# isl-org/Open3D-PointNet2-Semantic3D

Hardware: AMD Instinct MI355X
Metric: points/sec through SA+FP stack (B=16,N=8192) (higher is better)
Workload: dtype f32

## Files before the change

include/pn2_abi.h:

```cpp
#ifndef PN2_ABI_H_
#define PN2_ABI_H_

#include <stddef.h>
#include <stdint.h>

#ifdef __cplusplus
extern "C" {
#endif

#define PN2_ABI_VERSION 1

#define PN2_OK 0
#define PN2_EINVAL (-1)
#define PN2_ENULL (-2)
#define PN2_ERANGE (-3)
#define PN2_EUNSUP (-4)

#define PN2_ARITH_STRICT 0
#define PN2_ARITH_FMA 1
#define PN2_ARITH_FMA_ALT 2

int pn2_abi_version(void);
const char *pn2_build_info(void);
const char *pn2_strerror(int code);
// ... 207 lines not shown
                            double half_y, double scene_z_size, int cap, int *out_idx, int *out_cnt,
                            void *stream);

int pn2_scene_sample(int b, int npts, int cap, const double *points, const int *labels, const double *colors,
                     const int *idx, const int *cnt, const unsigned char *mask, double half_x, double half_y,
                     int *out_sel, float *out_centered, double *out_raw, int *out_labels, float *out_colors,
                     int *status, void *stream);

size_t pn2_voxel_downsample_workspace_bytes(int n);
int pn2_voxel_downsample(int n, const double *points, const double *colors, const int *labels, double voxel_size,
                         double *out_points, double *out_colors, int *out_labels, int *out_count, int *status,
                         void *workspace, size_t workspace_bytes, void *stream);

int pn2_dataset_workspace_size(int b, int max_chunks, unsigned long long *bytes);
int pn2_dataset_sample(int b, int npts, int num_scenes, int max_chunks, int use_color, int augment, const double *points,
                       const float *colors, const unsigned char *labels, const int *scene_offsets, const double *scene_cdf,
                       const double *scene_z_size, const float *label_weights, int num_label_weights, double half_x,
                       double half_y, unsigned long long seed, long long *counter, const int *draw_scene,
                       const int *draw_center, const unsigned char *draw_mask, int mask_cap, const double *draw_rot,
                       void *workspace, size_t workspace_bytes, int *out_info, double *out_finfo, int *out_sel,
                       float *out_data, int *out_labels, float *out_weights, void *stream);

int pn2_fp_mlp_fused_pre(int b, int n, int m, int c1, const float *dist, const int *idx, const float *points1,
                         const float *z, int nlayers, const int *widths, const float *const *w,
                         const float *const *bias, float *y, void *stream);
int pn2_fp_mlp_fused_pre_ld(int b, int n, int m, int c1, const float *dist, const int *idx, const float *points1,
                            int ld_points1, const float *z, int nlayers, const int *widths, const float *const *w,
                            const float *const *bias, float *y, void *stream);

int pn2_fp_mlp_fused_pre_schedule(int b, int n, int m, int c1, const float *dist, const int *idx, const float *points1,
                                  const float *z, int nlayers, const int *widths, const float *const *w,
                                  const float *const *bias, float *y, int schedule, void *stream);

int pn2_sa_mlp_fused_pre(int b, int n, int m, int nsample, const float *xyz, const float *new_xyz, const float *zf,
                         const int *idx, int nlayers, const int *widths, const float *const *w,
                         const float *const *bias, int pool, float *out, void *stream);

int pn2_fp_mlp_wide_pre(int b, int n, int m, int c1, const float *dist, const int *idx, const float *points1,
                        const float *z, int nlayers, const int *widths, const float *const *w,
                        const float *const *bias, float *y, void *stream);
int pn2_sa_mlp_wide_pre(int b, int n, int m, int nsample, const float *xyz, const float *new_xyz, const float *zf,
                        const int *idx, int nlayers, const int *widths, const float *const *w,
                        const float *const *bias, int pool, float *y, void *stream);

size_t pn2_ball_query_bin_bytes(int n);
int pn2_ball_query_bin(int b, int n, float radius, const float *xyz1, void *workspace, size_t workspace_bytes, void *stream);
int pn2_ball_query_bin_ld(int b, int n, float radius, const float *xyz1, int ld1, void *workspace, size_t workspace_bytes,
                          void *stream);
int pn2_query_ball_point_binned(int b, int n, int m, float radius, int nsample, const float *xyz1, const float *xyz2,
                                const void *bins, int *idx, int *pts_cnt, int arith_mode, void *stream);

int pn2_group_pool(long long rows, int k, int c, int mode, const float *x, const float *gxyz, float *out, void *stream);
int pn2_group_pool_grad(long long rows, int k, int c, int mode, const float *x, const float *gxyz, const float *dout,
                        float *dx, void *stream);

int pn2_bn_relu_forward_deferred(long long rows, int c, const float *y, const float *gamma, const float *beta,
                                 const float *bias, float eps, float decay, int stats_done, float *running_mean,
                                 float *running_var, void *workspace, size_t workspace_bytes, float *save_mean,
                                 float *save_invstd, float *scale, float *shift, void *stream);
int pn2_linear_bn_stats_xf(int rows, int cin, int cout, const float *x_raw, const float *w, float *y, void *bn_workspace,
                           size_t workspace_bytes, const float *a_scale, const float *a_shift, int a_relu, void *stream);
int pn2_linear_wgrad_accumulate_xf(int rows, int cin, int cout, const float *x_raw, const float *dy, float *dw,
                                   const float *a_scale, const float *a_shift, int a_relu, void *stream);

int pn2_linear_narrow(int rows, int cin, int cout, const float *x, const float *w, const float *bias, float *y, void *stream);

// ... 67 lines not shown
```

open3d-pointnet2-semantic3d_amd/_lib.py:

```python
import ctypes
import os
import sys

import torch

_HERE = os.path.dirname(os.path.abspath(__file__))
LIB_PATH = os.environ.get("PN2_HIP_LIBRARY") or os.path.join(_HERE, "libpn2_hip.so")

c_int, c_float, c_void_p = ctypes.c_int, ctypes.c_float, ctypes.c_void_p

SIGNATURES = {
    "pn2_farthest_point_sample": [c_int, c_int, c_int, c_void_p, c_void_p, c_void_p, c_int, c_void_p],
    "pn2_fps_gather": [c_int, c_int, c_int, c_void_p, c_void_p, c_void_p, c_void_p, c_int, c_void_p],
    "pn2_fps_nested": [c_int, c_int, c_int, c_void_p, c_void_p, c_void_p, c_void_p, c_void_p, c_void_p, c_int, c_void_p],
    "pn2_fps_nested_ld": [c_int, c_int, c_int, c_void_p, c_int, c_void_p, c_void_p, c_void_p, c_void_p, c_int, c_void_p],
    "pn2_coarse_geometry": [c_int, c_int, c_int, c_void_p, c_void_p, c_void_p, c_void_p, c_void_p, c_void_p, c_void_p, c_void_p,
                            c_void_p, c_void_p, c_void_p, c_void_p, c_int, c_int, c_void_p],
    "pn2_prob_sample": [c_int, c_int, c_int, c_void_p, c_void_p, c_void_p, c_void_p, c_void_p],
    "pn2_fps_large": [c_int, c_int, c_int, c_void_p, c_void_p, ctypes.c_size_t, c_void_p, c_void_p, c_int, c_void_p],
    "pn2_gather_point": [c_int, c_int, c_int, c_void_p, c_void_p, c_void_p, c_void_p],
    "pn2_gather_point_grad": [c_int, c_int, c_int, c_void_p, c_void_p, c_void_p, c_void_p],
    "pn2_query_ball_point": [c_int, c_int, c_int, c_float, c_int, c_void_p, c_void_p, c_void_p, c_void_p, c_int, c_void_p],
    "pn2_query_ball_point_ld": [c_int, c_int, c_int, c_float, c_int, c_void_p, c_int, c_void_p, c_void_p, c_void_p, c_int, c_void_p],
    "pn2_query_ball_point_kernel": [c_int, c_int, c_int, c_float, c_int, c_void_p, c_void_p, c_void_p, c_void_p, c_int, c_int,
                                    c_void_p],
    "pn2_query_ball_point_multi": [c_int, c_int, c_int, c_int, c_void_p, c_void_p, c_void_p, c_void_p, c_void_p, c_void_p,
                                   c_int, c_void_p],
    "pn2_selection_sort": [c_int, c_int, c_int, c_int, c_void_p, c_void_p, c_void_p, c_void_p],
    "pn2_group_point": [c_int, c_int, c_int, c_int, c_int, c_void_p, c_void_p, c_void_p, c_void_p],
    "pn2_group_point_grad": [c_int, c_int, c_int, c_int, c_int, c_void_p, c_void_p, c_void_p, c_void_p],
    "pn2_three_nn": [c_int, c_int, c_int, c_void_p, c_void_p, c_void_p, c_void_p, c_void_p],
    "pn2_three_nn_ld": [c_int, c_int, c_int, c_void_p, c_int, c_void_p, c_void_p, c_void_p, c_void_p],
    "pn2_three_interpolate": [c_int, c_int, c_int, c_int, c_void_p, c_void_p, c_void_p, c_void_p, c_void_p],
    "pn2_three_interpolate_grad": [c_int, c_int, c_int, c_int, c_void_p, c_void_p, c_void_p, c_void_p, c_void_p],
    "pn2_group_point_grad_ws": [c_int, c_int, c_int, c_int, c_int, c_void_p, c_void_p, c_void_p, c_void_p, ctypes.c_size_t,
                                c_void_p],
    "pn2_three_interpolate_grad_ws": [c_int, c_int, c_int, c_int, c_void_p, c_void_p, c_void_p, c_void_p, c_void_p,
                                      ctypes.c_size_t, c_void_p],
    "pn2_linear": [c_int, c_int, c_int, c_void_p, c_void_p, c_void_p, c_int, c_int, c_void_p, c_void_p],
    "pn2_linear_wgrad": [c_int, c_int, c_int, c_void_p, c_void_p, c_void_p, c_void_p],
    "pn2_bn_relu_forward": [ctypes.c_longlong, c_int, c_void_p, c_void_p, c_void_p, c_void_p, c_float, c_float, c_int, c_int,
                            c_void_p, c_void_p, c_void_p, ctypes.c_size_t, c_void_p, c_void_p, c_void_p, c_void_p, c_void_p],
    "pn2_bn_relu_backward": [ctypes.c_longlong, c_int, c_void_p, c_void_p, c_void_p, c_void_p, c_void_p, c_void_p, c_int,
                             c_int, c_void_p, c_void_p, c_void_p, ctypes.c_size_t, c_void_p, c_void_p, c_void_p, c_void_p],
    "pn2_sa_mlp_max_fused": [c_int, c_int, c_int, c_int, c_int, c_void_p, c_void_p, c_void_p, c_void_p,
                             c_int, c_void_p, c_void_p, c_void_p, c_void_p, c_void_p],
    "pn2_sa_mlp_max_fused_ld": [c_int, c_int, c_int, c_int, c_int, c_void_p, c_int, c_void_p, c_void_p, c_int, c_void_p,
                                c_int, c_void_p, c_void_p, c_void_p, c_void_p, c_void_p],
    "pn2_sa_mlp_max_fused_bf16": [c_int, c_int, c_int, c_int, c_int, c_void_p, c_void_p, c_void_p, c_void_p,
                                  c_int, c_void_p, c_void_p, c_void_p, c_void_p, c_void_p],
    "pn2_sa_mlp_rows_fused": [c_int, c_int, c_int, c_int, c_int, c_void_p, c_void_p, c_void_p, c_void_p,
                              c_int, c_void_p, c_void_p, c_void_p, c_void_p, c_void_p],
    "pn2_fp_interp_concat": [c_int, c_int, c_int, c_int, c_int, c_void_p, c_void_p, c_void_p, c_void_p,
                             c_void_p, c_int, c_void_p],
    "pn2_mlp_chain": [c_int, c_int, c_void_p, c_int, c_void_p, c_void_p, c_void_p, c_int, c_void_p, c_void_p],
    "pn2_fp_mlp_fused": [c_int, c_int, c_int, c_int, c_int, c_void_p, c_void_p, c_void_p, c_void_p,
                         c_int, c_void_p, c_void_p, c_void_p, c_void_p, c_void_p],
    "pn2_interpolate_label_with_color": [c_int, c_int, c_void_p, c_void_p, c_void_p, c_void_p, c_void_p, c_int, c_void_p,
                                         ctypes.c_size_t, c_void_p],
    "pn2_sa_group_concat": [c_int, c_int, c_int, c_int, c_int, c_void_p, c_void_p, c_void_p, c_void_p,
                            c_void_p, c_void_p],
    "pn2_bn_relu_forward_ws0": [ctypes.c_longlong, c_int, c_void_p, c_void_p, c_void_p, c_void_p, c_float, c_float, c_int, c_int,
                            c_void_p, c_void_p, c_void_p, ctypes.c_size_t, c_void_p, c_void_p, c_void_p, c_void_p, c_void_p],
    "pn2_bn_relu_backward_ws0": [ctypes.c_longlong, c_int, c_void_p, c_void_p, c_void_p, c_void_p, c_void_p, c_void_p, c_int,
                             c_int, c_void_p, c_void_p, c_void_p, ctypes.c_size_t, c_void_p, c_void_p, c_void_p, c_void_p],
    "pn2_mlp_wide": [c_int, c_int, c_int, c_void_p, c_int, c_void_p, c_void_p, c_void_p, c_int, c_int, c_void_p, c_void_p],
    "pn2_sa_mlp_wide": [c_int, c_int, c_int, c_int, c_int, c_void_p, c_void_p, c_void_p, c_void_p, c_int, c_void_p, c_void_p,
                        c_void_p, c_int, c_void_p, c_void_p],
    "pn2_fp_mlp_wide": [c_int, c_int, c_int, c_int, c_int, c_void_p, c_void_p, c_void_p, c_void_p, c_int, c_void_p, c_void_p,
                        c_void_p, c_void_p, c_void_p],
    "pn2_multi_copy": [c_int, c_void_p, c_void_p, c_void_p, c_void_p],
    "pn2_multi_copy_fill": [c_int, c_void_p, c_void_p, c_void_p, c_int, c_void_p, c_void_p, c_void_p, c_void_p],
    "pn2_scatter_plan_build": [c_int, c_int, c_int, c_int, c_void_p, c_void_p, c_int, c_void_p, ctypes.c_size_t, c_void_p],
    "pn2_scatter_plan_build_multi": [c_int, c_int, c_void_p, c_void_p, c_void_p, c_void_p, c_void_p, c_void_p, c_void_p, c_void_p,
                                     ctypes.c_size_t, c_void_p],
    "pn2_scatter_plan_apply": [c_int, c_int, c_int, c_int, c_int, c_void_p, c_int, c_void_p, ctypes.c_size_t, c_void_p, c_void_p],
    "pn2_linear_bn_stats": [c_int, c_int, c_int, c_void_p, c_void_p, c_void_p, c_void_p, ctypes.c_size_t, c_void_p],
# ... 266 lines not shown
```

open3d-pointnet2-semantic3d_amd/csrc/pn2_sa_fused.hip:

```cpp
#include "pn2_common.h"
#include <type_traits>
#include <utility>

namespace {

typedef float f32x4 __attribute__((ext_vector_type(4)));
typedef float f32x16 __attribute__((ext_vector_type(16)));

struct SaFusedParams {
    int n, m, c, groups;
    int kshift;
    int rows;
    int w[3];
    const float* xyz;
    const float* new_xyz;
    const float* points;
    const int* idx;
    const float* dist;
    const float* points1;
    int c1;
    int ldx, ldp, ld1;
    const float* W[3];
    const float* bias[3];
    float* out;
    int prio;
    int schedule;
#ifdef PN2_TUNING_HOOKS
    long long* stats;
    long long* trace;
    int tag;
#endif
};

#ifdef PN2_TUNING_HOOKS
#define PN2_CHAIN_STAMP(k_)                                                                                              \
    do {                                                                                                                 \
        if (p.stats && blockIdx.x < 4 && lane == 0 && (wave == 0 || wave == NW / 2) && tile_no < 4)                      \
            p.stats[((blockIdx.x * 2 + (wave ? 1 : 0)) * 4 + tile_no) * 8 + (k_)] = (long long)__builtin_readcyclecounter(); \
    } while (0)
#else
#define PN2_CHAIN_STAMP(k_) do { } while (0)
#endif

__device__ __forceinline__ int acc_chan(int r, int half) { return (r & 3) + 8 * (r >> 2) + 4 * half; }

__host__ __device__ inline int l1_steps(int c, bool vec8, bool dense = false, int c1 = 0) {
    return (dense ? 0 : 2) + (vec8 ? (c / 8) * 4 : (c + 1) / 2) + (c1 + 1) / 2;
}

__device__ __forceinline__ int l1_chan(int s, int h, int c, bool vec8, bool dense, int c1 = 0) {
    int base = 0;
    if (!dense) {
        if (s == 0) return h;
        if (s == 1) return h ? -1 : 2;
        s -= 2;
        base = 3;
    }
    const int nmain = vec8 ? (c / 8) * 4 : (c + 1) / 2;
// ... 111 lines not shown
        if (half == 0) orow[nt * 32 + l31] = v;
    }
}

template <int NT>
__device__ __forceinline__ void pool_store_k(const f32x16 (&acc)[NT], const float* __restrict__ sbias,
                                             float* __restrict__ out, int wout, int g, int kshift, int half, int l31) {
#pragma unroll
    for (int nt = 0; nt < NT; ++nt) {
        const float bv = sbias[nt * 32 + l31];
        if (kshift == 4) {
            float v0 = acc[nt][0], v1 = acc[nt][8];
#pragma unroll
            for (int r = 1; r < 8; ++r) { v0 = fmaxf(v0, acc[nt][r]); v1 = fmaxf(v1, acc[nt][8 + r]); }
            v0 = fmaxf(v0, __shfl_xor(v0, 32));
            v1 = fmaxf(v1, __shfl_xor(v1, 32));
            if (half == 0) {
                out[(size_t)(2 * g) * wout + nt * 32 + l31] = fmaxf(v0 + bv, 0.f);
                out[(size_t)(2 * g + 1) * wout + nt * 32 + l31] = fmaxf(v1 + bv, 0.f);
            }
        } else {
            float v = acc[nt][0];
#pragma unroll
            for (int r = 1; r < 16; ++r) v = fmaxf(v, acc[nt][r]);
            v = fmaxf(v, __shfl_xor(v, 32));
            v = fmaxf(v + bv, 0.f);
            if (half == 0)
                atomicMax(reinterpret_cast<int*>(out + (size_t)(g >> (kshift - 5)) * wout + nt * 32 + l31), __float_as_int(v));
        }
    }
}

template <int NT>
__device__ __forceinline__ void rows_store(const f32x16 (&acc)[NT], const float* __restrict__ sbias,
                                           float* __restrict__ obase, int wout, int row0, int rows,
                                           int half, int l31) {
    if (row0 + 32 <= rows) {
        float* __restrict__ o = obase + (size_t)(row0 + 4 * half) * wout + l31;
#pragma unroll
        for (int nt = 0; nt < NT; ++nt) {
            const float bv = sbias[nt * 32 + l31];
#pragma unroll
            for (int r = 0; r < 16; ++r)
                o[((r & 3) + 8 * (r >> 2)) * wout + nt * 32] = fmaxf(acc[nt][r] + bv, 0.f);
        }
        return;
    }
#pragma unroll
    for (int nt = 0; nt < NT; ++nt) {
        const float bv = sbias[nt * 32 + l31];
#pragma unroll
        for (int r = 0; r < 16; ++r) {
            const int row = row0 + acc_chan(r, half);
            if (row < rows) obase[(size_t)row * wout + nt * 32 + l31] = fmaxf(acc[nt][r] + bv, 0.f);
        }
    }
}

template <int NT>
__device__ __forceinline__ void rows_store_pk(const f32x16 (&acc)[NT], const float* __restrict__ sbias, float* __restrict__ obase,
                                              int wout, int row0, int rows, int half, int l31) {
    if (row0 + 32 > rows) { rows_store<NT>(acc, sbias, obase, wout, row0, rows, half, l31); return; }
    float* __restrict__ oq[4];
#pragma unroll
    for (int q = 0; q < 4; ++q) oq[q] = obase + (size_t)(row0 + 4 * half + 8 * q) * wout + l31;
#pragma unroll
    for (int nt = 0; nt < NT; ++nt) {
        const float bv = sbias[nt * 32 + l31];
        const f32x2 b2 = {bv, bv};
#pragma unroll
        for (int r = 0; r < 16; r += 2) {
            const f32x2 v = f32x2{acc[nt][r], acc[nt][r + 1]} + b2;
            oq[r >> 2][(r & 3) * wout + nt * 32] = fmaxf(v[0], 0.f);
            oq[r >> 2][((r + 1) & 3) * wout + nt * 32] = fmaxf(v[1], 0.f);
        }
    }
}

template <int L, int NT1, int NT2, int NT3, bool VEC8, bool DENSE, bool POOL, int NW, bool INTERP = false, bool PREZ = false>
__global__ void __launch_bounds__(NW * 64, (NW >= 8 ? NW / 4 : 2))
sa_fused_kernel(SaFusedParams p) {
    extern __shared__ __attribute__((aligned(16))) float smem[];
    const int tid = threadIdx.x;
    const int lane = tid & 63;
    const int half = lane >> 5;
    const int l31 = lane & 31;
    const int wave = __builtin_amdgcn_readfirstlane(tid >> 6);
    constexpr int W1 = NT1 * 32, W2 = NT2 * 32, W3 = NT3 * 32;
    const int c = PREZ ? 0 : p.c;
    const int c1 = INTERP ? p.c1 : 0;
    const int steps1 = l1_steps(c, VEC8, DENSE, c1);
    constexpr int NTH = NW * 64;

    int tile_no = 0;
    (void)tile_no;
    PN2_CHAIN_STAMP(0);
#ifdef PN2_TUNING_HOOKS
    const bool stagger = NW == 8 && L >= 2 && p.prio != 0;
#else
    constexpr bool stagger = false;
#endif
    float* wp1 = smem;
    float* wp2 = wp1 + steps1 * 2 * W1;
    float* wp3 = wp2 + (L >= 2 ? W1 * W2 : 0);
    float* sb1 = wp3 + (L >= 3 ? W2 * W3 : 0);
    float* sb2 = sb1 + W1;
    float* sb3 = sb2 + (L >= 2 ? W2 : 0);
    int* stagger_flag = reinterpret_cast<int*>(sb3 + (L >= 3 ? W3 : 0));
    if (stagger && tid < NW) stagger_flag[tid] = 0;
    auto stage4 = [&](float* dst, int count4, const float* __restrict__ src, auto index_of, int ntw) {
        const int W = ntw * 32;
        for (int base = 0; base < count4; base += NTH * 8) {
            f32x4 v[8];
#pragma unroll
            for (int u = 0; u < 8; ++u) {
                const int e = base + u * NTH + tid;
                const int gi = e < count4 ? index_of(e) : -1;
                const f32x4 t = *reinterpret_cast<const f32x4*>(src + (gi >= 0 ? gi : 0));
                const f32x4 z = {0.f, 0.f, 0.f, 0.f};
                v[u] = gi >= 0 ? t : z;
            }
#pragma unroll
            for (int u = 0; u < 8; ++u) {
                const int e = base + u * NTH + tid;
                if (e < count4) {
                    if (ntw == 1) {
                        *reinterpret_cast<f32x4*>(dst + e * 4) = v[u];
                    } else {
                        const int col = (e % (W / 4)) * 4, sh = e / (W / 4);
                        float* __restrict__ d = dst + sh * W + (col & 31) * ntw + (col >> 5);
#pragma unroll
                        for (int j = 0; j < 4; ++j) d[j * ntw] = v[u][j];
                    }
                }
            }
        }
    };
    auto stage1 = [&](float* dst, int count, const float* __restrict__ src) {
        for (int e = tid; e < count; e += NTH) dst[e] = src[e];
    };
    stage4(wp1, steps1 * 2 * W1 / 4, p.W[0], [&](int e4) {
        const int col = (e4 % (W1 / 4)) * 4, sh = e4 / (W1 / 4);
        const int ch = l1_chan(sh >> 1, sh & 1, c, VEC8, DENSE, c1);
        return ch >= 0 ? ch * W1 + col : -1;
    }, NT1);
    stage1(sb1, W1, p.bias[0]);
    if constexpr (L >= 2) {
        stage4(wp2, W1 * W2 / 4, p.W[1], [&](int e4) {
            const int col = (e4 % (W2 / 4)) * 4, sh = e4 / (W2 / 4);
            const int s = sh >> 1, h = sh & 1;
            return ((s >> 4) * 32 + acc_chan(s & 15, h)) * W2 + col;
        }, NT2);
        stage1(sb2, W2, p.bias[1]);
    }
    if constexpr (L >= 3) {
        stage4(wp3, W2 * W3 / 4, p.W[2], [&](int e4) {
            const int col = (e4 % (W3 / 4)) * 4, sh = e4 / (W3 / 4);
            const int s = sh >> 1, h = sh & 1;
            return ((s >> 4) * 32 + acc_chan(s & 15, h)) * W3 + col;
        }, NT3);
        stage1(sb3, W3, p.bias[2]);
    }
    __syncthreads();
    PN2_CHAIN_STAMP(1);

    constexpr int WOUT = L == 1 ? W1 : (L == 2 ? W2 : W3);
    int g_lo = blockIdx.x * NW + wave, g_hi = p.groups, g_step = gridDim.x * NW;
    if ((gridDim.x & 7u) == 0u && (p.groups & 7) == 0) {
        const int per = p.groups >> 3, xcd = blockIdx.x & 7, slot = blockIdx.x >> 3;
        g_lo = xcd * per + slot * NW + wave;
        g_hi = (xcd + 1) * per;
        g_step = (gridDim.x >> 3) * NW;
    }
    for (int g = g_lo; g < g_hi; g += g_step, ++tile_no) {
        PN2_CHAIN_STAMP(2);
        size_t prow;
        f32x16 a1[NT1];
        zero_acc<NT1>(a1);
        constexpr bool LAST1 = (L == 1);
        const float* w1l = wp1 + half * W1 + l31 * NT1;
        constexpr int S0 = DENSE ? 0 : 2;
        if constexpr (DENSE) {
            const int row = g * 32 + l31;
            prow = (size_t)(row < p.rows ? row : p.rows - 1);
        } else {
            const int grp = (g * 32 + l31) >> p.kshift;
            const int bi = grp / p.m;
            const int ii = p.idx[(size_t)g * 32 + l31];
            prow = (size_t)bi * p.n + ii;
            const float cxv = p.new_xyz[(size_t)grp * 3 + 0];
            const float cyv = p.new_xyz[(size_t)grp * 3 + 1];
            const float czv = p.new_xyz[(size_t)grp * 3 + 2];
            const float rx = p.xyz[prow * p.ldx + 0] - cxv;
            const float ry = p.xyz[prow * p.ldx + 1] - cyv;
            const float rz = p.xyz[prow * p.ldx + 2] - czv;
            mfma_step<NT1, LAST1>(a1, w1l + 0 * 2 * W1, half ? ry : rx);
            mfma_step<NT1, LAST1>(a1, w1l + 1 * 2 * W1, half ? 0.f : rz);
        }
        if constexpr (INTERP) {
            const float* __restrict__ dr = p.dist + prow * 3;
            const int* __restrict__ ir = p.idx + prow * 3;
            const float d1 = fmaxf(dr[0], 1e-10f), d2 = fmaxf(dr[1], 1e-10f), d3 = fmaxf(dr[2], 1e-10f);
            const float r1 = 1.0f / d1, r2 = 1.0f / d2, r3 = 1.0f / d3;
            const float norm = (r1 + r2) + r3;
            const float w1 = r1 / norm, w2 = r2 / norm, w3 = r3 / norm;
            const size_t kb = (prow / (size_t)p.n) * (size_t)p.m;
            if constexpr (PREZ) {
                const f32x4* __restrict__ z1 = reinterpret_cast<const f32x4*>(p.points + (kb + ir[0]) * W1) + half;
                const f32x4* __restrict__ z2 = reinterpret_cast<const f32x4*>(p.points + (kb + ir[1]) * W1) + half;
                const f32x4* __restrict__ z3 = reinterpret_cast<const f32x4*>(p.points + (kb + ir[2]) * W1) + half;
                if (c1 > 0) {
                    const float* __restrict__ fp = p.points1 + prow * p.ld1;
                    const int ns = (c1 + 1) >> 1;
                    for (int sp = 0; sp < ns; ++sp) {
                        const int ch = 2 * sp + half;
                        const float v = ch < c1 ? fp[ch] : 0.f;
                        mfma_step<NT1, LAST1>(a1, w1l + sp * 2 * W1, v);
                    }
                }
#pragma unroll
                for (int nt = 0; nt < NT1; ++nt) {
// ... 61 lines not shown
            f32x4 cur = fp[0];
            float wq[4][NT1];
#pragma unroll
            for (int q = 0; q < 4; ++q) load_w<NT1>(wq[q], w1l + (S0 + q) * 2 * W1);
            for (int t = 0; t < nt8; ++t) {
                const f32x4 nxt = fp[(t + 1 < nt8 ? t + 1 : t) * 2];
#pragma unroll
                for (int q = 0; q < 4; ++q) {
                    mfma_regs<NT1, LAST1>(a1, wq[q], cur[q]);
                    __builtin_amdgcn_sched_barrier(0);
                    const int sn = S0 + 4 * (t + 1) + q;
                    load_w<NT1>(wq[q], w1l + (sn < steps1 ? sn : steps1 - 1) * 2 * W1);
                    __builtin_amdgcn_sched_barrier(0);
                }
                cur = nxt;
            }
        } else {
            const float* __restrict__ fp = p.points + prow * p.ldp;
            const int ns = (c + 1) >> 1;
            for (int sp = 0; sp < ns; ++sp) {
                const int ch = 2 * sp + half;
                const float v = ch < c ? fp[ch] : 0.f;
                mfma_step<NT1, LAST1>(a1, w1l + (S0 + sp) * 2 * W1, v);
            }
        }
        float* __restrict__ orow = p.out + (size_t)g * WOUT;
        PN2_CHAIN_STAMP(3);
        if (stagger && tile_no == 0 && wave >= NW / 2) {
            while (__hip_atomic_load(&stagger_flag[wave - NW / 2], __ATOMIC_RELAXED, __HIP_MEMORY_SCOPE_WORKGROUP) == 0)
                __builtin_amdgcn_s_sleep(8);
        }
        if constexpr (L == 1) {
            if constexpr (POOL) {
                if (DENSE || p.kshift == 5) pool_store<NT1>(a1, sb1, orow, half, l31);
                else pool_store_k<NT1>(a1, sb1, p.out, WOUT, g, p.kshift, half, l31);
            }
            else rows_store<NT1>(a1, sb1, p.out, WOUT, g * 32, p.rows, half, l31);
        } else {
            bias_relu_T_pk<NT1>(a1, sb1 + 4 * half);
            f32x16 a2[NT2];
            zero_acc<NT2>(a2);
            layer_from_regs<NT1, NT2, L == 2>(a1, a2, wp2, W2, half, l31);
            PN2_CHAIN_STAMP(4);
            if (L == 2 && stagger && tile_no == 0 && wave < NW / 2 && lane == 0)
                __hip_atomic_store(&stagger_flag[wave], 1, __ATOMIC_RELAXED, __HIP_MEMORY_SCOPE_WORKGROUP);
            if constexpr (L == 2) {
                if constexpr (POOL) {
                if (DENSE || p.kshift == 5) pool_store<NT2>(a2, sb2, orow, half, l31);
                else pool_store_k<NT2>(a2, sb2, p.out, WOUT, g, p.kshift, half, l31);
            }
                else rows_store<NT2>(a2, sb2, p.out, WOUT, g * 32, p.rows, half, l31);
            } else {
                bias_relu_T_pk<NT2>(a2, sb2 + 4 * half);
                f32x16 a3[NT3];
                zero_acc<NT3>(a3);
                layer_from_regs<NT2, NT3, true>(a2, a3, wp3, W3, half, l31);
                PN2_CHAIN_STAMP(5);
                if (stagger && tile_no == 0 && wave < NW / 2 && lane == 0)
                    __hip_atomic_store(&stagger_flag[wave], 1, __ATOMIC_RELAXED, __HIP_MEMORY_SCOPE_WORKGROUP);
                if constexpr (POOL) {
                if (DENSE || p.kshift == 5) pool_store<NT3>(a3, sb3, orow, half, l31);
                else pool_store_k<NT3>(a3, sb3, p.out, WOUT, g, p.kshift, half, l31);
            }
                else rows_store<NT3>(a3, sb3, p.out, WOUT, g * 32, p.rows, half, l31);
            }
        }
        PN2_CHAIN_STAMP(6);
    }
    if (stagger && wave < NW / 2 && lane == 0)
        __hip_atomic_store(&stagger_flag[wave], 1, __ATOMIC_RELAXED, __HIP_MEMORY_SCOPE_WORKGROUP);
}

template <int... I, class F>
__device__ __forceinline__ void static_for_impl(std::integer_sequence<int, I...>, F&& f) { (f(std::integral_constant<int, I>{}), ...); }
template <int N, class F>
__device__ __forceinline__ void static_for(F&& f) { static_for_impl(std::make_integer_sequence<int, N>{}, f); }

constexpr int kPipeSkipSteps = 4;

template <int NT2, int NT3, int NS>
__global__ void __launch_bounds__(256, 1)
fp_chain_pipe_kernel(SaFusedParams p) {
    extern __shared__ __attribute__((aligned(16))) float smem[];
    constexpr int NW = 4, NTH = 256, NT1 = 4;
    const int tid = threadIdx.x;
    const int lane = tid & 63;
    const int half = lane >> 5;
    const int l31 = lane & 31;
    const int wave = __builtin_amdgcn_readfirstlane(tid >> 6);
    constexpr int W1 = NT1 * 32, W2 = NT2 * 32, W3 = NT3 * 32;
    static_assert(NT2 == 4 && NT3 == 4, "side-job schedule written for three 128-wide layers");
    const int c1 = p.c1;
    constexpr int steps1 = NS;
    float* wp1 = smem;
    float* wp2 = wp1 + steps1 * 2 * W1;
    float* wp3 = wp2 + W1 * W2;
    float* sb1 = wp3 + W2 * W3;
    float* sb2 = sb1 + W1;
    float* sb3 = sb2 + W2;
    int tile_no = 0;
// ... 212 lines not shown
        PN2_CHAIN_STAMP(6);
        ++tile_no;
    }
#ifdef PN2_TUNING_HOOKS
    if (p.stats && lane == 0) {
        p.stats[256 + blockIdx.x * NW + wave] = (long long)__builtin_readcyclecounter() - t_begin;
        unsigned hwid;
        asm volatile("s_getreg_b32 %0, hwreg(HW_REG_HW_ID)" : "=s"(hwid));
        unsigned xcc;
        asm volatile("s_getreg_b32 %0, hwreg(HW_REG_XCC_ID)" : "=s"(xcc));
        p.stats[256 + 1024 + blockIdx.x * NW + wave] = ((long long)xcc << 32) | hwid;
        p.stats[256 + 2048 + blockIdx.x * NW + wave] = (long long)__builtin_amdgcn_s_memrealtime();
        p.stats[256 + 3072 + blockIdx.x * NW + wave] = t_real0;
    }
    if (p.trace && lane == 0) {
        const int wv = blockIdx.x * NW + wave;
        unsigned long long* cnt = reinterpret_cast<unsigned long long*>(p.trace) + (size_t)p.tag * 1024 + wv;
        const unsigned long long cidx = atomicAdd(cnt, 1ull);
        long long* r = p.trace + 8 * 1024 + (((size_t)p.tag * 1024 + wv) * 16 + (cidx & 15ull)) * 2;
        r[0] = t_real0;
        r[1] = (long long)__builtin_amdgcn_s_memrealtime();
    }
#endif
}

PN2_TUNABLE(int, g_chain_prio, 0)
PN2_TUNABLE(long long*, g_chain_stats, nullptr)
PN2_TUNABLE(int, g_chain_nw, 0)
PN2_TUNABLE(int, g_chain_pipe, 1)
PN2_TUNABLE(int, g_chain_grid, 256)
PN2_TUNABLE(long long*, g_chain_trace, nullptr)
PN2_TUNABLE(int, g_chain_tag, 0)

template <int L, int NT1, int NT2, int NT3, bool VEC8, bool DENSE, bool POOL, bool INTERP = false, bool PREZ = false>
int launch_chain(const SaFusedParams& p_in, hipStream_t st) {
    SaFusedParams p = p_in;
    p.prio = g_chain_prio;
    if (!p.ldx) p.ldx = 3;
    if (!p.ldp) p.ldp = p.c;
    if (!p.ld1) p.ld1 = p.c1;
#ifdef PN2_TUNING_HOOKS
    p.stats = g_chain_stats;
    p.trace = g_chain_trace;
    p.tag = g_chain_tag & 7;
#endif
    constexpr int W1 = NT1 * 32, W2 = NT2 * 32, W3 = NT3 * 32;
    const int steps1 = l1_steps(PREZ ? 0 : p.c, VEC8, DENSE, INTERP ? p.c1 : 0);
    size_t floats = (size_t)steps1 * 2 * W1 + W1;
    if (L >= 2) floats += (size_t)W1 * W2 + W2;
    if (L >= 3) floats += (size_t)W2 * W3 + W3;
    const size_t bytes = floats * sizeof(float) + 64;
    if (bytes > 150 * 1024) return PN2_EUNSUP;
    const int need4 = (p.groups + 3) / 4;
    if constexpr (L == 1) {
        if (g_chain_nw == 16 && p.groups >= 4096) {
            auto kern = sa_fused_kernel<L, NT1, NT2, NT3, VEC8, DENSE, POOL, 16, INTERP, PREZ>;
            static bool attr_set = false;
            if (!attr_set) {
                hipError_t e = hipFuncSetAttribute(reinterpret_cast<const void*>(kern),
                                                   hipFuncAttributeMaxDynamicSharedMemorySize, 160 * 1024);
                if (e != hipSuccess) return (int)e;
                attr_set = true;
            }
            kern<<<g_chain_grid, 1024, bytes, st>>>(p);
            PN2_RETURN_IF_LAUNCH_FAILED();
            return PN2_OK;
        }
    }
    if constexpr (L == 3 && INTERP && PREZ && DENSE && !POOL && NT1 == 4) {
// ... 11 lines not shown
            }
            const size_t pbytes = ((size_t)(ns2 ? 2 : 4) * 2 * W1 + W1 + (size_t)W1 * W2 + W2 + (size_t)W2 * W3 + W3) * sizeof(float);
            int grid = g_chain_grid;
            if (grid > need4) grid = need4;
            kern<<<grid, 256, pbytes, st>>>(p);
            PN2_RETURN_IF_LAUNCH_FAILED();
            return PN2_OK;
        }
    }
    if constexpr (L == 3 && INTERP && PREZ) {
#ifdef PN2_FP4_NW12
        constexpr bool nw12 = true;
#else
        const bool nw12 = g_chain_nw == 12;
#endif
        if (nw12 && bytes > 78 * 1024 && p.groups >= 2048) {
            auto kern = sa_fused_kernel<L, NT1, NT2, NT3, VEC8, DENSE, POOL, 12, INTERP, PREZ>;
            static bool attr_set = false;
            if (!attr_set) {
                hipError_t e = hipFuncSetAttribute(reinterpret_cast<const void*>(kern),
                                                   hipFuncAttributeMaxDynamicSharedMemorySize, 160 * 1024);
                if (e != hipSuccess) return (int)e;
                attr_set = true;
            }
            int grid = g_chain_grid;
            const int need12 = (p.groups + 11) / 12;
            if (grid > need12) grid = need12;
            kern<<<grid, 768, bytes, st>>>(p);
            PN2_RETURN_IF_LAUNCH_FAILED();
            return PN2_OK;
        }
    }
    if (bytes > 78 * 1024 && p.groups >= 2048 && g_chain_nw != 4) {
        auto kern = sa_fused_kernel<L, NT1, NT2, NT3, VEC8, DENSE, POOL, 8, INTERP, PREZ>;
        static bool attr_set = false;
        if (!attr_set) {
            hipError_t e = hipFuncSetAttribute(reinterpret_cast<const void*>(kern),
                                               hipFuncAttributeMaxDynamicSharedMemorySize, 160 * 1024);
            if (e != hipSuccess) return (int)e;
            attr_set = true;
        }
        int grid = g_chain_grid;
        const int need8 = (p.groups + 7) / 8;
        if (grid > need8) grid = need8;
        kern<<<grid, 512, bytes, st>>>(p);
    } else {
        auto kern = sa_fused_kernel<L, NT1, NT2, NT3, VEC8, DENSE, POOL, 4, INTERP, PREZ>;
        static bool attr_set = false;
        if (!attr_set) {
            hipError_t e = hipFuncSetAttribute(reinterpret_cast<const void*>(kern),
                                               hipFuncAttributeMaxDynamicSharedMemorySize, 160 * 1024);
            if (e != hipSuccess) return (int)e;
            attr_set = true;
        }
        int grid = bytes > 78 * 1024 ? g_chain_grid : g_chain_grid * 2;
        if (grid > need4) grid = need4;
        kern<<<grid, 256, bytes, st>>>(p);
    }
    PN2_RETURN_IF_LAUNCH_FAILED();
    return PN2_OK;
}

}

#ifdef PN2_TUNING_HOOKS
extern "C" int pn2_debug_set_chain_stats(long long* dev_ptr) { g_chain_stats = dev_ptr; return 0; }
extern "C" int pn2_debug_set_chain_trace(long long* dev_ptr) { g_chain_trace = dev_ptr; return 0; }
extern "C" int pn2_debug_set_fused(int what, int value) {
    if (what == 6) { g_chain_grid = value; return 0; }
    if (what == 7) { g_chain_nw = value; return 0; }
    if (what == 13) { g_chain_prio = value; return 0; }
    if (what == 14) { g_chain_pipe = value; return 0; }
    if (what == 16) { g_chain_tag = value; return 0; }
    return PN2_EINVAL;
}
#endif

static int sa_fused_impl(int b, int n, int m, int nsample, int c, const float* xyz,
                         const float* new_xyz, const float* points, const int* idx,
                         int nlayers, const int* widths, const float* const* w,
                         const float* const* bias, float* out, bool pool, void* stream, int ld_xyz, int ld_points);

extern "C" int pn2_sa_mlp_max_fused(int b, int n, int m, int nsample, int c, const float* xyz,
                                    const float* new_xyz, const float* points, const int* idx,
                                    int nlayers, const int* widths, const float* const* w,
                                    const float* const* bias, float* out, void* stream) {
    return sa_fused_impl(b, n, m, nsample, c, xyz, new_xyz, points, idx, nlayers, widths, w, bias, out, true, stream, 3, c);
}

extern "C" int pn2_sa_mlp_max_fused_ld(int b, int n, int m, int nsample, int c, const float* xyz, int ld_xyz,
                                       const float* new_xyz, const float* points, int ld_points, const int* idx,
                                       int nlayers, const int* widths, const float* const* w,
                                       const float* const* bias, float* out, void* stream) {
    return sa_fused_impl(b, n, m, nsample, c, xyz, new_xyz, points, idx, nlayers, widths, w, bias, out, true, stream, ld_xyz,
                         c > 0 ? ld_points : 0);
}

extern "C" int pn2_sa_mlp_rows_fused(int b, int n, int m, int nsample, int c, const float* xyz,
                                     const float* new_xyz, const float* points, const int* idx,
                                     int nlayers, const int* widths, const float* const* w,
                                     const float* const* bias, float* out, void* stream) {
    return sa_fused_impl(b, n, m, nsample, c, xyz, new_xyz, points, idx, nlayers, widths, w, bias, out, false, stream, 3, c);
}

static int sa_fused_impl(int b, int n, int m, int nsample, int c, const float* xyz,
                         const float* new_xyz, const float* points, const int* idx,
                         int nlayers, const int* widths, const float* const* w,
                         const float* const* bias, float* out, bool pool, void* stream, int ld_xyz, int ld_points) {
    if (b <= 0 || n <= 0 || m <= 0 || nsample <= 0 || c < 0 || nlayers <= 0) return PN2_EINVAL;
// ... 208 lines not shown
```

open3d-pointnet2-semantic3d_amd/util/pointnet_util.py:

```python

import torch

from . import tf_util
from .._lib import float_array, int_array, launch, lib, ptr, ptr_table, require_cuda, rows_in_place, u64_array
from ..tf_ops import tf_grouping
from ..tf_ops.tf_grouping import query_ball_point_multi, group_point, knn_point, query_ball_point
from ..tf_ops.tf_interpolate import three_interpolate, three_nn
from ..tf_ops.tf_sampling import (farthest_point_sample, farthest_point_sample_and_gather, farthest_point_sample_with_ties,
                                  gather_point, tag_fps_output)


def sample_and_group(npoint, radius, nsample, xyz, points, knn=False, use_xyz=True, geometry=None):
    plan = None
    if geometry is not None:
        new_xyz, idx = geometry[0], geometry[1]
        plan = geometry[2] if len(geometry) > 2 else None
    else:
        fps_idx, fps_tie, _ = farthest_point_sample_with_ties(npoint, xyz)
        new_xyz = tag_fps_output(gather_point(xyz, fps_idx), fps_tie)
        if knn:
            _, idx = knn_point(nsample, xyz, new_xyz)
        else:
            idx, pts_cnt = query_ball_point(radius, nsample, xyz, new_xyz)
    if USE_FUSED_TRAIN_FRONT and points is not None and use_xyz and points.dtype == torch.float32:
# ... 20 lines not shown
    new_xyz = torch.zeros((b, 1, 3), dtype=torch.float32, device=xyz.device)
    idx = torch.arange(n, dtype=torch.int32, device=xyz.device).reshape(1, 1, n).repeat(b, 1, 1)
    grouped_xyz = xyz.reshape(b, 1, n, 3)
    if points is not None:
        new_points = torch.cat([xyz, points], dim=2) if use_xyz else points
        new_points = new_points.unsqueeze(1)
    else:
        new_points = grouped_xyz
    return new_xyz, new_points, idx, grouped_xyz


def _sa_fused_inference(xyz, new_xyz, points, idx, mlp, bn, conv_scope_fmt, pool=True, xyz_last=False):
    b, n, _ = xyz.shape
    m, nsample = idx.shape[1], idx.shape[2]
    c = 0 if points is None else points.shape[2]
    bf16 = points is not None and points.dtype == torch.bfloat16
    if bf16:
        if not pool or nsample not in (32, 64) or c % 16 != 0:
            return None
    elif nsample != 32 and (not pool or nsample not in (16, 64, 128, 256)):
        return None
    if len(mlp) > 3 or any(w % 32 != 0 or w > 128 for w in mlp):
        return None
    ws, bs = [], []
    cin = 3 + c
    for i, cout in enumerate(mlp):
        with tf_util.variable_scope(conv_scope_fmt % i):
            w2, b2 = tf_util.folded_dense(cin, cout, bn, (1, 1, cin, cout),
                                          rotate_rows=3 if (xyz_last and i == 0 and c > 0) else 0)
        ws.append(w2)
        bs.append(b2)
        cin = cout
    L = len(mlp)
    widths, bptrs = int_array(mlp), ptr_table(bs)
    oshape = (b, m, mlp[-1]) if pool else (b, m, nsample, mlp[-1])
    out = torch.empty(oshape, dtype=torch.float32, device=xyz.device)
    if (USE_HOISTED_SA and not bf16 and nsample == 32 and c >= 32 and c % 4 == 0
            and ((pool and tuple(mlp) in ((64, 64, 128), (128, 128, 128))) or (not pool and tuple(mlp) == (128, 128)))):
        w1x, w1f = tf_util.split_first_layer(ws[0], 3, c, "sa_pre")
        xyz, points = xyz.contiguous(), points.contiguous()
        zf = tf_util.hoist_gemm(points.reshape(b * n, c), w1f)
        if launch("pn2_sa_mlp_fused_pre", xyz, b, n, m, nsample, ptr(xyz), ptr(new_xyz), ptr(zf), ptr(idx), L, widths,
                  ptr_table([w1x] + ws[1:]), bptrs, int(bool(pool)), ptr(out), may_refuse=True):
            return out
    wptrs = ptr_table(ws)
    xyz_v, ldx = rows_in_place(xyz)
    pts, ldp = (None, 0) if points is None else rows_in_place(points)
    if pool and not bf16 and (ldx != 3 or (points is not None and ldp != c)):
        if launch("pn2_sa_mlp_max_fused_ld", xyz, b, n, m, nsample, c, ptr(xyz_v), ldx, ptr(new_xyz), ptr(pts), ldp, ptr(idx), L,
                  widths, wptrs, bptrs, ptr(out), may_refuse=True):
            return out
    xyz_v = xyz_v.contiguous()
    pts = None if pts is None else pts.contiguous()
    name = "pn2_sa_mlp_max_fused_bf16" if bf16 else ("pn2_sa_mlp_max_fused" if pool else "pn2_sa_mlp_rows_fused")
    ok = launch(name, xyz, b, n, m, nsample, c, ptr(xyz_v), ptr(new_xyz), ptr(pts), ptr(idx), L, widths, wptrs, bptrs, ptr(out),
                may_refuse=True)
    return out if ok else None


def _sa_group_concat(xyz, new_xyz, points, idx):
    b, n, _ = xyz.shape
    m, nsample = idx.shape[1], idx.shape[2]
    c = 0 if points is None else points.shape[2]
    out = torch.empty((b, m, nsample, 3 + c), dtype=torch.float32, device=xyz.device)
    pts = None if points is None else points.contiguous()
    launch("pn2_sa_group_concat", xyz, b, n, m, nsample, c, ptr(xyz), ptr(new_xyz), ptr(pts), ptr(idx), ptr(out))
# ... 77 lines not shown


class _FPInterpConcat(torch.autograd.Function):

    @staticmethod
    def forward(ctx, dist, idx, points1, points2, plan=None):
        out = _fp_interp_concat(dist, idx, points1, points2)
        ctx.save_for_backward(dist, idx, plan)
        ctx.m, ctx.c2 = points2.shape[1], points2.shape[2]
        ctx.c1 = 0 if points1 is None else points1.shape[2]
        return out

    @staticmethod
    def backward(ctx, grad_out):
        dist, idx, plan = ctx.saved_tensors
        g1 = grad_out[..., ctx.c2:] if ctx.c1 and ctx.needs_input_grad[2] else None
        if not ctx.needs_input_grad[3]:
            return None, None, g1, None, None
        if _plan_usable(plan, ctx.c2):
            n = idx.shape[1]
            return None, None, g1, _scatter_plan_apply(plan, grad_out, 0, ctx.c2, 3 * n, 3, ctx.m), None
        d = torch.clamp(dist, min=1e-10)
        w = (1.0 / d)
        w = (w / w.sum(dim=2, keepdim=True)).contiguous()
        from ..tf_ops.tf_interpolate import three_interpolate_grad
        g2 = three_interpolate_grad(grad_out[..., :ctx.c2].contiguous(), idx, w, ctx.m)
        return None, None, g1, g2, None


USE_FUSED_SA = True


USE_HOISTED_SA = True
USE_HOISTED_FP = True
def sa_geometry(xyz, npoint, radius, nsample):
    _, new_xyz = farthest_point_sample_and_gather(npoint, xyz)
    idx, _ = query_ball_point(radius, nsample, xyz, new_xyz)
    return new_xyz, idx


USE_COARSE_GEOMETRY = True
COARSE_MAX_N, COARSE_MAX_LEVELS, COARSE_MAX_NN_M = 1024, 4, 256


def coarse_geometry_fits(n0, npoints, want_nn=True):
    if not USE_COARSE_GEOMETRY or not (0 < n0 <= COARSE_MAX_N) or not (0 < len(npoints) <= COARSE_MAX_LEVELS):
        return False
    n = n0
    for m in npoints:
        if not (0 < m <= n) or (want_nn and not (3 <= m <= COARSE_MAX_NN_M)):
            return False
        n = m
    return True


def coarse_geometry(xyz0, npoints, radii, nsamples, want_nn=True, fps_arith_mode=None, bq_arith_mode=None):
    from .. import config
    from ..tf_ops.tf_sampling import fps_tie_record
    require_cuda(xyz0)
    if xyz0.dim() != 3 or xyz0.shape[2] != 3 or xyz0.dtype != torch.float32:
        raise ValueError("coarse_geometry expects (batch_size,num_points,3) float32 xyz0")
    nlev = len(npoints)
    if not (len(radii) == len(nsamples) == nlev):
        raise ValueError("coarse_geometry expects one radius and one nsample per level")
    tie_in = fps_tie_record(xyz0, fps_arith_mode)
    xyz0 = xyz0.detach().contiguous()
# ... 361 lines not shown
```

Before: 345.8 million.

## Pack ball-query groups with few distinct neighbours into shared MFMA row tiles

In the pooled SA fused kernel, each block first classifies its groups by how many leading idx entries are distinct. Groups whose live neighbours fit in 8 or 16 rows are packed four or two to a 32-row MFMA tile, and the pooling store reduces per sub-group. Ball-query padding repeats the first index, so padded rows do not change the max, and the packing is meant to skip redundant MLP work on them. It adds a classification pass, extra LDS, block-level persistent looping with syncthreads, and a runtime toggle that defaults to on.

```diff
diff --git a/include/pn2_abi.h b/include/pn2_abi.h
--- a/include/pn2_abi.h
+++ b/include/pn2_abi.h
@@ -263,6 +263,8 @@
                                   const float *z, int nlayers, const int *widths, const float *const *w,
                                   const float *const *bias, float *y, int schedule, void *stream);
 
+int pn2_set_sa_row_packing(int on);
+
 int pn2_sa_mlp_fused_pre(int b, int n, int m, int nsample, const float *xyz, const float *new_xyz, const float *zf,
                          const int *idx, int nlayers, const int *widths, const float *const *w,
                          const float *const *bias, int pool, float *out, void *stream);
diff --git a/open3d-pointnet2-semantic3d_amd/_lib.py b/open3d-pointnet2-semantic3d_amd/_lib.py
--- a/open3d-pointnet2-semantic3d_amd/_lib.py
+++ b/open3d-pointnet2-semantic3d_amd/_lib.py
@@ -43,6 +43,7 @@
                             c_void_p, c_void_p, c_void_p, ctypes.c_size_t, c_void_p, c_void_p, c_void_p, c_void_p, c_void_p],
     "pn2_bn_relu_backward": [ctypes.c_longlong, c_int, c_void_p, c_void_p, c_void_p, c_void_p, c_void_p, c_void_p, c_int,
                              c_int, c_void_p, c_void_p, c_void_p, ctypes.c_size_t, c_void_p, c_void_p, c_void_p, c_void_p],
+    "pn2_set_sa_row_packing": [c_int],
     "pn2_sa_mlp_max_fused": [c_int, c_int, c_int, c_int, c_int, c_void_p, c_void_p, c_void_p, c_void_p,
                              c_int, c_void_p, c_void_p, c_void_p, c_void_p, c_void_p],
     "pn2_sa_mlp_max_fused_ld": [c_int, c_int, c_int, c_int, c_int, c_void_p, c_int, c_void_p, c_void_p, c_int, c_void_p,
diff --git a/open3d-pointnet2-semantic3d_amd/csrc/pn2_sa_fused.hip b/open3d-pointnet2-semantic3d_amd/csrc/pn2_sa_fused.hip
--- a/open3d-pointnet2-semantic3d_amd/csrc/pn2_sa_fused.hip
+++ b/open3d-pointnet2-semantic3d_amd/csrc/pn2_sa_fused.hip
@@ -1,4 +1,5 @@
 #include "pn2_common.h"
+#include <atomic>
 #include <type_traits>
 #include <utility>
 
@@ -24,6 +25,7 @@
     const float* bias[3];
     float* out;
     int prio;
+    int blk;
     int schedule;
 #ifdef PN2_TUNING_HOOKS
     long long* stats;
@@ -201,6 +203,37 @@
 }
 
 template <int NT>
+__device__ __forceinline__ void pool_store_packed(const f32x16 (&acc)[NT], const float* __restrict__ sbias, float* __restrict__ out,
+                                                  int wout, int sshift, int nvalid, const int (&gq)[4], int half, int l31) {
+#pragma unroll
+    for (int nt = 0; nt < NT; ++nt) {
+        const float bv = sbias[nt * 32 + l31];
+        float v[4];
+#pragma unroll
+        for (int q = 0; q < 4; ++q)
+            v[q] = fmaxf(fmaxf(acc[nt][4 * q], acc[nt][4 * q + 1]), fmaxf(acc[nt][4 * q + 2], acc[nt][4 * q + 3]));
+        if (sshift == 3) {
+#pragma unroll
+            for (int q = 0; q < 4; ++q) {
+                const float u = fmaxf(v[q], __shfl_xor(v[q], 32));
+                if (half == 0 && q < nvalid) out[(size_t)gq[q] * wout + nt * 32 + l31] = fmaxf(u + bv, 0.f);
+            }
+        } else if (sshift == 4) {
+#pragma unroll
+            for (int q = 0; q < 2; ++q) {
+                float u = fmaxf(v[2 * q], v[2 * q + 1]);
+                u = fmaxf(u, __shfl_xor(u, 32));
+                if (half == 0 && q < nvalid) out[(size_t)gq[q] * wout + nt * 32 + l31] = fmaxf(u + bv, 0.f);
+            }
+        } else {
+            float u = fmaxf(fmaxf(v[0], v[1]), fmaxf(v[2], v[3]));
+            u = fmaxf(u, __shfl_xor(u, 32));
+            if (half == 0) out[(size_t)gq[0] * wout + nt * 32 + l31] = fmaxf(u + bv, 0.f);
+        }
+    }
+}
+
+template <int NT>
 __device__ __forceinline__ void rows_store(const f32x16 (&acc)[NT], const float* __restrict__ sbias,
                                            float* __restrict__ obase, int wout, int row0, int rows,
                                            int half, int l31) {
@@ -246,9 +279,11 @@
     }
 }
 
-template <int L, int NT1, int NT2, int NT3, bool VEC8, bool DENSE, bool POOL, int NW, bool INTERP = false, bool PREZ = false>
+template <int L, int NT1, int NT2, int NT3, bool VEC8, bool DENSE, bool POOL, int NW, bool INTERP = false, bool PREZ = false,
+          bool PACK = false>
 __global__ void __launch_bounds__(NW * 64, (NW >= 8 ? NW / 4 : 2))
 sa_fused_kernel(SaFusedParams p) {
+    static_assert(!PACK || (POOL && !DENSE && !INTERP), "PACK: the pooled gather mode only");
     extern __shared__ __attribute__((aligned(16))) float smem[];
     const int tid = threadIdx.x;
     const int lane = tid & 63;
@@ -265,7 +300,7 @@
     (void)tile_no;
     PN2_CHAIN_STAMP(0);
 #ifdef PN2_TUNING_HOOKS
-    const bool stagger = NW == 8 && L >= 2 && p.prio != 0;
+    const bool stagger = NW == 8 && L >= 2 && p.prio != 0 && !PACK;
 #else
     constexpr bool stagger = false;
 #endif
@@ -277,6 +312,9 @@
     float* sb3 = sb2 + (L >= 2 ? W2 : 0);
     int* stagger_flag = reinterpret_cast<int*>(sb3 + (L >= 3 ? W3 : 0));
     if (stagger && tid < NW) stagger_flag[tid] = 0;
+    int* s_cls = stagger_flag + 16;
+    int* s_desc = s_cls + 64;
+    (void)s_cls; (void)s_desc;
     auto stage4 = [&](float* dst, int count4, const float* __restrict__ src, auto index_of, int ntw) {
         const int W = ntw * 32;
         for (int base = 0; base < count4; base += NTH * 8) {
@@ -341,9 +379,58 @@
         g_hi = (xcd + 1) * per;
         g_step = (gridDim.x >> 3) * NW;
     }
+    int pk_b = 0, pk_nb = 0, pk_bstep = 1, pk_lo = 0, pk_hi = 0;
+    if constexpr (PACK) {
+        pk_lo = 0; pk_hi = p.groups; pk_b = blockIdx.x; pk_bstep = gridDim.x;
+        if ((gridDim.x & 7u) == 0u && (p.groups & 7) == 0) {
+            const int per = p.groups >> 3, xcd = blockIdx.x & 7;
+            pk_lo = xcd * per; pk_hi = pk_lo + per; pk_b = blockIdx.x >> 3; pk_bstep = gridDim.x >> 3;
+        }
+        pk_nb = (pk_hi - pk_lo + p.blk - 1) / p.blk;
+    }
+    for (bool pk_first = true;; pk_b += pk_bstep, pk_first = false) {
+    int pk_base = 0, pk_n32 = 0, pk_t16 = 0, pk_n16 = 0, pk_n8 = 0;
+    if constexpr (PACK) {
+        if (pk_b >= pk_nb) break;
+        if (!pk_first) __syncthreads();
+        pk_base = pk_lo + pk_b * p.blk;
+        const int cnt = min(p.blk, pk_hi - pk_base);
+        for (int c0 = 2 * wave; c0 < cnt; c0 += 2 * NW) {
+            const int cl = c0 + half;
+            const int v = p.idx[(size_t)(pk_base + (cl < cnt ? cl : c0)) * 32 + l31];
+            const int first = __shfl(v, lane & 32);
+            const unsigned long long diff = __ballot(v != first);
+            const unsigned mine = (unsigned)(diff >> (lane & 32));
+            const int live = 32 - __clz(mine | 1u);
+            if (l31 == 0 && cl < cnt) s_cls[cl] = live <= 8 ? 8 : (live <= 16 ? 16 : 32);
+        }
+        __syncthreads();
+        const int cls = lane < cnt ? s_cls[lane] : 0;
+        const unsigned long long m32 = __ballot(cls == 32), m16 = __ballot(cls == 16), m8 = __ballot(cls == 8);
+        const int n16 = __popcll(m16), n8 = __popcll(m8);
+        const int promote = ((n16 & 1) && (n8 & 3) == 1) ? 1 : 0;
+        pk_n32 = __popcll(m32); pk_n16 = n16 + promote; pk_n8 = n8 - promote;
+        pk_t16 = (pk_n16 + 1) >> 1;
+        if (wave == 0 && lane < cnt) {
+            const unsigned long long below = (1ull << lane) - 1ull;
+            int tile, slot;
+            if (cls == 32) { tile = __popcll(m32 & below); slot = 0; }
+            else {
+                int c = cls, r = __popcll((cls == 16 ? m16 : m8) & below);
+                if (promote && c == 8 && r == n8 - 1) { c = 16; r = n16; }
+                if (c == 16) { tile = pk_n32 + (r >> 1); slot = r & 1; }
+                else { tile = pk_n32 + pk_t16 + (r >> 2); slot = r & 3; }
+            }
+            s_desc[tile * 4 + slot] = pk_base + lane;
+        }
+        __syncthreads();
+        g_lo = wave; g_hi = pk_n32 + pk_t16 + ((pk_n8 + 3) >> 2); g_step = NW;
+    }
     for (int g = g_lo; g < g_hi; g += g_step, ++tile_no) {
         PN2_CHAIN_STAMP(2);
         size_t prow;
+        int pk_sshift = 5, pk_nvalid = 1, pk_gq[4] = {0, 0, 0, 0};
+        (void)pk_sshift; (void)pk_nvalid; (void)pk_gq;
         f32x16 a1[NT1];
         zero_acc<NT1>(a1);
         constexpr bool LAST1 = (L == 1);
@@ -353,9 +440,21 @@
             const int row = g * 32 + l31;
             prow = (size_t)(row < p.rows ? row : p.rows - 1);
         } else {
-            const int grp = (g * 32 + l31) >> p.kshift;
+            int grp, ii;
+            if constexpr (PACK) {
+                if (g < pk_n32) { pk_sshift = 5; pk_nvalid = 1; }
+                else if (g < pk_n32 + pk_t16) { pk_sshift = 4; pk_nvalid = min(2, pk_n16 - 2 * (g - pk_n32)); }
+                else { pk_sshift = 3; pk_nvalid = min(4, pk_n8 - 4 * (g - pk_n32 - pk_t16)); }
+#pragma unroll
+                for (int q = 0; q < 4; ++q) pk_gq[q] = __builtin_amdgcn_readfirstlane(s_desc[g * 4 + (q < pk_nvalid ? q : 0)]);
+                const int q = l31 >> pk_sshift;
+                grp = q == 1 ? pk_gq[1] : (q == 2 ? pk_gq[2] : (q == 3 ? pk_gq[3] : pk_gq[0]));
+                ii = p.idx[(size_t)grp * 32 + (l31 & ((1 << pk_sshift) - 1))];
+            } else {
+                grp = (g * 32 + l31) >> p.kshift;
+                ii = p.idx[(size_t)g * 32 + l31];
+            }
             const int bi = grp / p.m;
-            const int ii = p.idx[(size_t)g * 32 + l31];
             prow = (size_t)bi * p.n + ii;
             const float cxv = p.new_xyz[(size_t)grp * 3 + 0];
             const float cyv = p.new_xyz[(size_t)grp * 3 + 1];
@@ -483,7 +582,8 @@
         }
         if constexpr (L == 1) {
             if constexpr (POOL) {
-                if (DENSE || p.kshift == 5) pool_store<NT1>(a1, sb1, orow, half, l31);
+                if constexpr (PACK) pool_store_packed<NT1>(a1, sb1, p.out, WOUT, pk_sshift, pk_nvalid, pk_gq, half, l31);
+                else if (DENSE || p.kshift == 5) pool_store<NT1>(a1, sb1, orow, half, l31);
                 else pool_store_k<NT1>(a1, sb1, p.out, WOUT, g, p.kshift, half, l31);
             }
             else rows_store<NT1>(a1, sb1, p.out, WOUT, g * 32, p.rows, half, l31);
@@ -497,7 +597,8 @@
                 __hip_atomic_store(&stagger_flag[wave], 1, __ATOMIC_RELAXED, __HIP_MEMORY_SCOPE_WORKGROUP);
             if constexpr (L == 2) {
                 if constexpr (POOL) {
-                if (DENSE || p.kshift == 5) pool_store<NT2>(a2, sb2, orow, half, l31);
+                if constexpr (PACK) pool_store_packed<NT2>(a2, sb2, p.out, WOUT, pk_sshift, pk_nvalid, pk_gq, half, l31);
+                else if (DENSE || p.kshift == 5) pool_store<NT2>(a2, sb2, orow, half, l31);
                 else pool_store_k<NT2>(a2, sb2, p.out, WOUT, g, p.kshift, half, l31);
             }
                 else rows_store<NT2>(a2, sb2, p.out, WOUT, g * 32, p.rows, half, l31);
@@ -510,13 +611,16 @@
                 if (stagger && tile_no == 0 && wave < NW / 2 && lane == 0)
                     __hip_atomic_store(&stagger_flag[wave], 1, __ATOMIC_RELAXED, __HIP_MEMORY_SCOPE_WORKGROUP);
                 if constexpr (POOL) {
-                if (DENSE || p.kshift == 5) pool_store<NT3>(a3, sb3, orow, half, l31);
+                if constexpr (PACK) pool_store_packed<NT3>(a3, sb3, p.out, WOUT, pk_sshift, pk_nvalid, pk_gq, half, l31);
+                else if (DENSE || p.kshift == 5) pool_store<NT3>(a3, sb3, orow, half, l31);
                 else pool_store_k<NT3>(a3, sb3, p.out, WOUT, g, p.kshift, half, l31);
             }
                 else rows_store<NT3>(a3, sb3, p.out, WOUT, g * 32, p.rows, half, l31);
             }
         }
         PN2_CHAIN_STAMP(6);
+    }
+    if constexpr (!PACK) break;
     }
     if (stagger && wave < NW / 2 && lane == 0)
         __hip_atomic_store(&stagger_flag[wave], 1, __ATOMIC_RELAXED, __HIP_MEMORY_SCOPE_WORKGROUP);
@@ -795,9 +899,28 @@
 PN2_TUNABLE(long long*, g_chain_trace, nullptr)
 PN2_TUNABLE(int, g_chain_tag, 0)
 
+std::atomic<int> g_sa_row_packing{1};
+constexpr size_t kPackLdsBytes = (64 + 64 * 4) * sizeof(int);
+
+template <int L, int NT1, int NT2, int NT3, bool VEC8, bool DENSE, bool POOL, int NW, bool INTERP, bool PREZ>
+auto chain_kernel(bool pack) -> void (*)(SaFusedParams) {
+    if constexpr (POOL && !DENSE && !INTERP) {
+        if (pack) return sa_fused_kernel<L, NT1, NT2, NT3, VEC8, DENSE, POOL, NW, INTERP, PREZ, true>;
+    }
+    return sa_fused_kernel<L, NT1, NT2, NT3, VEC8, DENSE, POOL, NW, INTERP, PREZ, false>;
+}
+
+inline int pack_block(int groups, int grid) {
+    int per = groups, nsl = grid;
+    if ((grid & 7) == 0 && (groups & 7) == 0) { per = groups >> 3; nsl = grid >> 3; }
+    const int blk = (per + nsl - 1) / nsl;
+    return blk < 1 ? 1 : (blk > 64 ? 64 : blk);
+}
+
 template <int L, int NT1, int NT2, int NT3, bool VEC8, bool DENSE, bool POOL, bool INTERP = false, bool PREZ = false>
 int launch_chain(const SaFusedParams& p_in, hipStream_t st) {
     SaFusedParams p = p_in;
+    const bool pack = POOL && !DENSE && !INTERP && p.kshift == 5 && g_sa_row_packing.load(std::memory_order_relaxed) != 0;
     p.prio = g_chain_prio;
     if (!p.ldx) p.ldx = 3;
     if (!p.ldp) p.ldp = p.c;
@@ -875,30 +998,32 @@
         }
     }
     if (bytes > 78 * 1024 && p.groups >= 2048 && g_chain_nw != 4) {
-        auto kern = sa_fused_kernel<L, NT1, NT2, NT3, VEC8, DENSE, POOL, 8, INTERP, PREZ>;
-        static bool attr_set = false;
-        if (!attr_set) {
+        auto kern = chain_kernel<L, NT1, NT2, NT3, VEC8, DENSE, POOL, 8, INTERP, PREZ>(pack);
+        static bool attr_set[2] = {false, false};
+        if (!attr_set[pack]) {
             hipError_t e = hipFuncSetAttribute(reinterpret_cast<const void*>(kern),
                                                hipFuncAttributeMaxDynamicSharedMemorySize, 160 * 1024);
             if (e != hipSuccess) return (int)e;
-            attr_set = true;
+            attr_set[pack] = true;
         }
         int grid = g_chain_grid;
         const int need8 = (p.groups + 7) / 8;
         if (grid > need8) grid = need8;
-        kern<<<grid, 512, bytes, st>>>(p);
+        p.blk = pack_block(p.groups, grid);
+        kern<<<grid, 512, bytes + (pack ? kPackLdsBytes : 0), st>>>(p);
     } else {
-        auto kern = sa_fused_kernel<L, NT1, NT2, NT3, VEC8, DENSE, POOL, 4, INTERP, PREZ>;
-        static bool attr_set = false;
-        if (!attr_set) {
+        auto kern = chain_kernel<L, NT1, NT2, NT3, VEC8, DENSE, POOL, 4, INTERP, PREZ>(pack);
+        static bool attr_set[2] = {false, false};
+        if (!attr_set[pack]) {
             hipError_t e = hipFuncSetAttribute(reinterpret_cast<const void*>(kern),
                                                hipFuncAttributeMaxDynamicSharedMemorySize, 160 * 1024);
             if (e != hipSuccess) return (int)e;
-            attr_set = true;
+            attr_set[pack] = true;
         }
         int grid = bytes > 78 * 1024 ? g_chain_grid : g_chain_grid * 2;
         if (grid > need4) grid = need4;
-        kern<<<grid, 256, bytes, st>>>(p);
+        p.blk = pack_block(p.groups, grid);
+        kern<<<grid, 256, bytes + (pack ? kPackLdsBytes : 0), st>>>(p);
     }
     PN2_RETURN_IF_LAUNCH_FAILED();
     return PN2_OK;
@@ -918,6 +1043,11 @@
     return PN2_EINVAL;
 }
 #endif
+
+extern "C" int pn2_set_sa_row_packing(int on) {
+    g_sa_row_packing.store(on != 0, std::memory_order_relaxed);
+    return PN2_OK;
+}
 
 static int sa_fused_impl(int b, int n, int m, int nsample, int c, const float* xyz,
                          const float* new_xyz, const float* points, const int* idx,
diff --git a/open3d-pointnet2-semantic3d_amd/util/pointnet_util.py b/open3d-pointnet2-semantic3d_amd/util/pointnet_util.py
--- a/open3d-pointnet2-semantic3d_amd/util/pointnet_util.py
+++ b/open3d-pointnet2-semantic3d_amd/util/pointnet_util.py
@@ -76,6 +76,7 @@
         bs.append(b2)
         cin = cout
     L = len(mlp)
+    _sync_sa_row_packing(xyz)
     widths, bptrs = int_array(mlp), ptr_table(bs)
     oshape = (b, m, mlp[-1]) if pool else (b, m, nsample, mlp[-1])
     out = torch.empty(oshape, dtype=torch.float32, device=xyz.device)
@@ -219,6 +220,18 @@
 
 
 USE_HOISTED_SA = True
+USE_SA_ROW_PACKING = True
+_sa_row_packing_told = True
+
+
+def _sync_sa_row_packing(where):
+    global _sa_row_packing_told
+    want = bool(USE_SA_ROW_PACKING)
+    if want != _sa_row_packing_told:
+        launch("pn2_set_sa_row_packing", where, int(want), stream=False)
+        _sa_row_packing_told = want
+
+
 USE_HOISTED_FP = True
 def sa_geometry(xyz, npoint, radius, nsample):
     _, new_xyz = farthest_point_sample_and_gather(npoint, xyz)
```

New measurement: 369.9 million (median of 6 runs). 1.07x the previous value.
